# yl-jiang/YOLOSeries

Measured on AMD Instinct MI355X. Metric: images/sec (640x640) YOLOv5s train-step, higher is better.
Workload: dtype bf16; 1 GPU; YOLOv5s bf16 train step (fwd+loss+bwd+clip+SGD+EMA), batch 64/GPU x 640x640 synthetic COCO-80, random-init (BASELINE.json configs[1]); global_batch=64, parallelism=dp1

## Files before the change

yoloseries_amd/csrc/conv_dg2.hip:

```cpp
#include "common.h"
#include <stdlib.h>

namespace {

typedef __attribute__((ext_vector_type(4))) unsigned int u32x4_t;
typedef unsigned int u32x4_nt __attribute__((ext_vector_type(4)));

__device__ __forceinline__ uint4 dg_ld_nt16(const uint16_t* p) {
    u32x4_nt v = __builtin_nontemporal_load(reinterpret_cast<const u32x4_nt*>(p));
    return make_uint4(v.x, v.y, v.z, v.w);
}
__device__ __forceinline__ void dg_st_nt16(uint16_t* p, uint4 v) {
    u32x4_nt w = {v.x, v.y, v.z, v.w};
    __builtin_nontemporal_store(w, reinterpret_cast<u32x4_nt*>(p));
}

constexpr int DG_RPX1 = 128;
constexpr int dg_pmax(int pt) { return pt == 1 ? 168 : 304; }

struct Dg2K {
    const uint16_t* gz; int ldg, Nk;
    const uint16_t* w; int Ktot;
    uint16_t* out; int ld0, C;
    int B, Hg, Wg, Ho, Wo;
    int TH, TW, tx, ty, ntiles, nchunk, npatch;
    int accumulate;
    const uint16_t* z; int ldz; const float* ws; int wsC; float* part;
    unsigned gzbytes, wbytes;
};

template <int CT, int KC, int PT>
constexpr int dg_smem_bytes() {
    const int main_b = (dg_pmax(PT) + 9 * 32 * CT) * (KC + 8) * 2;
    const int stg_b = 2 * DG_RPX1 * PT * (32 * CT + 8) * 2;
    return (main_b > stg_b ? main_b : stg_b) + 2 * 32 * CT * 4;
}

template <int CT, int KC, int EPI, int PT>
__global__ __launch_bounds__(256 * CT, 1) void conv_dg2_kernel(const Dg2K p)
{
    constexpr int NT = 256 * CT;
    constexpr int DG_RPX = DG_RPX1 * PT;
    constexpr int DG_PMAX = dg_pmax(PT);
    constexpr int PITCH = KC + 8;
    constexpr int CHR = KC / 8;
    constexpr int CB = 32 * CT;
    constexpr int PPP = NT / CHR;
    constexpr int NPI = (DG_PMAX + PPP - 1) / PPP;
    constexpr int NWI = (9 * CB + PPP - 1) / PPP;
    constexpr int SP = CB + 8;
    constexpr int CPR = CB / 8;
    constexpr int NOI = 2 * DG_RPX * CPR / NT;
    constexpr unsigned OOB = 0x80000000u;
    constexpr int PATCH_BYTES = DG_PMAX * PITCH * 2;
    constexpr int STG_BYTES = 2 * DG_RPX * SP * 2;
    constexpr bool STG_IN_PATCH = STG_BYTES <= PATCH_BYTES;
    static_assert(NT % CPR == 0 && NOI == 4 * PT, "read-out mapping");

    extern __shared__ __attribute__((aligned(16))) unsigned char smem[];
    uint16_t* sP = reinterpret_cast<uint16_t*>(smem);
    uint16_t* sW = sP + DG_PMAX * PITCH;
    float* sStat = reinterpret_cast<float*>(smem + dg_smem_bytes<CT, KC, PT>() - 2 * CB * 4);
    uint16_t* sStg = reinterpret_cast<uint16_t*>(smem);

    const int t = threadIdx.x;
    const int lane = t & 63;
    const int wave = t >> 6;
    const int wq = wave & 3, wct = wave >> 2;
    const int c0 = blockIdx.y * CB;
    const int TWp = p.TW + 1;

    const __amdgpu_buffer_rsrc_t rsg = __builtin_amdgcn_make_buffer_rsrc((void*)p.gz, 0, p.gzbytes, 0x00020000);
    const __amdgpu_buffer_rsrc_t rsw = __builtin_amdgcn_make_buffer_rsrc((void*)p.w, 0, p.wbytes, 0x00020000);

    const int ch = t % CHR, row0 = t / CHR;
    unsigned woff[NWI];
#pragma unroll
    for (int j = 0; j < NWI; ++j) {
        const int row = row0 + j * PPP;
        const int tap = row / CB, c = row - tap * CB;
        woff[j] = row < 9 * CB ? (unsigned)((((size_t)(c0 + c) * p.Ktot) + tap * p.Nk + ch * 8) * 2) : OOB;
    }
    int ppij[NPI];
#pragma unroll
    for (int j = 0; j < NPI; ++j) {
        const int pp = row0 + j * PPP;
        const int pi = pp / TWp;
        ppij[j] = pp < p.npatch ? (pi << 8) | (pp - pi * TWp) : -1;
    }
    const int koff = (lane >> 5) * 8;
    int rpx[PT];
    const uint16_t* xbase[PT];
#pragma unroll
    for (int pt = 0; pt < PT; ++pt) {
        rpx[pt] = (wq * PT + pt) * 32 + (lane & 31);
        const bool rvalid = rpx[pt] < p.TH * p.TW;
        const int ri = rvalid ? rpx[pt] / p.TW : 0;
        const int rj = rvalid ? rpx[pt] - ri * p.TW : 0;
        xbase[pt] = sP + (ri * TWp + rj) * PITCH + koff;
    }
    const uint16_t* const wbase = sW + (wct * 32 + (lane & 31)) * PITCH + koff;

    if (EPI == 3) {
        for (int i = t; i < 2 * CB; i += NT) {
            const int which = i / CB, c = i - which * CB;
            sStat[i] = (c0 + c < p.C) ? p.ws[(size_t)which * p.wsC + c0 + c] : 0.f;
        }
    }
    float bs_[8], bq_[8];
#pragma unroll
    for (int e = 0; e < 8; ++e) { bs_[e] = 0.f; bq_[e] = 0.f; }

    u32x4_t rp[NPI], rw[NWI];
    const bool w_resident = STG_IN_PATCH && p.nchunk == 1;

    auto tile_origin = [&](int tile, int& b, int& i0, int& j0) {
        const int per = p.tx * p.ty;
        b = tile / per;
        const int r = tile - b * per;
        const int tyi = r / p.tx;
        i0 = tyi * p.TH; j0 = (r - tyi * p.tx) * p.TW;
    };
    auto load_regs = [&](int tile, int kc, bool with_w) {
        int b, i0, j0;
        tile_origin(tile, b, i0, j0);
        const int so = kc * KC * 2;
#pragma unroll
        for (int j = 0; j < NPI; ++j) {
            const int gi = i0 + (ppij[j] >> 8), gj = j0 + (ppij[j] & 0xff);
            const bool ok = ppij[j] >= 0 && gi < p.Hg && gj < p.Wg;
            const unsigned off = ok ? (unsigned)(((b * p.Hg + gi) * p.Wg + gj) * (p.ldg * 2) + ch * 16) : OOB;
            rp[j] = __builtin_amdgcn_raw_buffer_load_b128(rsg, off, so, 0);
        }
        if (with_w) {
#pragma unroll
            for (int j = 0; j < NWI; ++j) rw[j] = __builtin_amdgcn_raw_buffer_load_b128(rsw, woff[j], so, 0);
        }
    };
    auto store_regs = [&](bool with_w) {
        uint16_t* dp = sP + row0 * PITCH + ch * 8;
#pragma unroll
        for (int j = 0; j < NPI; ++j)
            if (row0 + j * PPP < DG_PMAX) *reinterpret_cast<u32x4_t*>(dp + j * PPP * PITCH) = rp[j];
        if (with_w) {
            uint16_t* dw = sW + row0 * PITCH + ch * 8;
#pragma unroll
            for (int j = 0; j < NWI; ++j)
                if (row0 + j * PPP < 9 * CB) *reinterpret_cast<u32x4_t*>(dw + j * PPP * PITCH) = rw[j];
        }
    };

    f32x16_t acc[4][PT];
    int tile = blockIdx.x;
    if (tile >= p.ntiles) return;
    load_regs(tile, 0, true);
    bool first = true;
    for (; tile < p.ntiles; tile += gridDim.x) {
#pragma unroll
        for (int q = 0; q < 4; ++q)
#pragma unroll
            for (int pt = 0; pt < PT; ++pt)
#pragma unroll
                for (int r = 0; r < 16; ++r) acc[q][pt][r] = 0.f;
        for (int kc = 0; kc < p.nchunk; ++kc) {
            const bool with_w = !w_resident || first;
            __syncthreads();
            store_regs(with_w);
            __syncthreads();
            first = false;
            {
                int nt = tile, nk = kc + 1;
                if (nk == p.nchunk) { nk = 0; nt = tile + gridDim.x; }
                if (nt < p.ntiles) load_regs(nt, nk, !w_resident);
            }
#pragma unroll
            for (int sh = 0; sh < 4; ++sh) {
                const int dy = sh >> 1, dx = sh & 1;
                bf16x8_t xf[PT][KC / 16];
#pragma unroll
                for (int pt = 0; pt < PT; ++pt)
#pragma unroll
                    for (int ks = 0; ks < KC / 16; ++ks)
                        xf[pt][ks] = __builtin_bit_cast(bf16x8_t, *reinterpret_cast<const uint4*>(xbase[pt] + (dy * TWp + dx) * PITCH + ks * 16));
#pragma unroll
                for (int a = 0; a < (dy ? 1 : 2); ++a) {
                    const int kh = dy ? 0 : 1 + a;
#pragma unroll
                    for (int b2 = 0; b2 < (dx ? 1 : 2); ++b2) {
                        const int kw = dx ? 0 : 1 + b2;
                        const int tap = kh * 3 + kw;
                        const int cls = (kh != 1 ? 2 : 0) + (kw != 1 ? 1 : 0);
#pragma unroll
                        for (int ks = 0; ks < KC / 16; ++ks) {
                            const bf16x8_t wf = __builtin_bit_cast(bf16x8_t, *reinterpret_cast<const uint4*>(wbase + tap * CB * PITCH + ks * 16));
#pragma unroll
                            for (int pt = 0; pt < PT; ++pt)
                                acc[cls][pt] = __builtin_amdgcn_mfma_f32_32x32x16_bf16(wf, xf[pt][ks], acc[cls][pt], 0, 0, 0);
                        }
                    }
                }
            }
        }

        int b, i0, j0;
        tile_origin(tile, b, i0, j0);
        const int cch = t % CPR;
        const int n = c0 + cch * 8;
#pragma unroll
        for (int ph = 0; ph < 2; ++ph) {
            int oidx[NOI];
            constexpr bool ZPRE = EPI == 3 && PT == 1;
            uint4 zpre[ZPRE ? NOI : 1];
#pragma unroll
            for (int it = 0; it < NOI; ++it) {
                const int row = t / CPR + it * (NT / CPR);
                const int r = row >> 1, pw = row & 1;
                const int i = r / p.TW, j = r - i * p.TW;
                const int gi = i0 + i, gj = j0 + j;
                const bool ok = r < p.TH * p.TW && gi < p.Hg && gj < p.Wg && n < p.C;
                oidx[it] = ok ? (b * p.Ho + 2 * gi + ph) * p.Wo + 2 * gj + pw : -1;
                if (ZPRE) {
                    zpre[it] = make_uint4(0, 0, 0, 0);
                    if (ok) zpre[it] = dg_ld_nt16(p.z + (size_t)oidx[it] * p.ldz + n);
                }
            }
            __syncthreads();
#pragma unroll
            for (int pw = 0; pw < 2; ++pw)
#pragma unroll
                for (int pt = 0; pt < PT; ++pt) {
                    uint16_t* dst = sStg + (rpx[pt] * 2 + pw) * SP + wct * 32 + 4 * (lane >> 5);
                    const f32x16_t& a = acc[ph * 2 + pw][pt];
#pragma unroll
                    for (int q = 0; q < 4; ++q) {
                        uint2 v;
                        v.x = pack2(a[4 * q + 0], a[4 * q + 1]);
                        v.y = pack2(a[4 * q + 2], a[4 * q + 3]);
                        *reinterpret_cast<uint2*>(dst + 8 * q) = v;
                    }
                }
            __syncthreads();
#pragma unroll
            for (int it = 0; it < NOI; ++it) {
                if (oidx[it] < 0) continue;
                const int row = t / CPR + it * (NT / CPR);
                uint4 v = *reinterpret_cast<const uint4*>(sStg + row * SP + cch * 8);
                uint16_t* dst = p.out + (size_t)oidx[it] * p.ld0 + n;
                if (p.accumulate) {
                    const uint4 ov = *reinterpret_cast<const uint4*>(dst);
                    float f[8], g0[8];
                    unpack8(v, f);
                    unpack8(ov, g0);
#pragma unroll
                    for (int e = 0; e < 8; ++e) f[e] += g0[e];
                    v = pack8(f);
                }
                if (EPI == 3) dg_st_nt16(dst, v);
                else *reinterpret_cast<uint4*>(dst) = v;
                if (EPI == 3) {
                    float g[8], z[8];
                    unpack8(v, g);
                    const uint4 zv = ZPRE ? zpre[it] : dg_ld_nt16(p.z + (size_t)oidx[it] * p.ldz + n);
                    unpack8(zv, z);
                    const float4 s0 = *reinterpret_cast<const float4*>(sStat + cch * 8);
                    const float4 s1 = *reinterpret_cast<const float4*>(sStat + cch * 8 + 4);
                    const float4 h0 = *reinterpret_cast<const float4*>(sStat + CB + cch * 8);
                    const float4 h1 = *reinterpret_cast<const float4*>(sStat + CB + cch * 8 + 4);
                    const float sc[8] = {s0.x, s0.y, s0.z, s0.w, s1.x, s1.y, s1.z, s1.w};
                    const float sh[8] = {h0.x, h0.y, h0.z, h0.w, h1.x, h1.y, h1.z, h1.w};
#pragma unroll
                    for (int e = 0; e < 8; ++e) {
                        const float a = z[e] * sc[e] + sh[e];
                        const float sg = sigmoid_fast(a);
                        const float dz = g[e] * (sg * (1.f + a * (1.f - sg)));
                        bs_[e] += dz; bq_[e] += dz * z[e];
                    }
                }
            }
        }
    }

    if (EPI == 3) {
        float* sRed = reinterpret_cast<float*>(smem);
        __syncthreads();
#pragma unroll
        for (int e = 0; e < 8; ++e) { sRed[t * 16 + e] = bs_[e]; sRed[t * 16 + 8 + e] = bq_[e]; }
        __syncthreads();
        for (int i = t; i < 2 * CB; i += NT) {
            const int which = i / CB, c = i - which * CB;
            float v = 0.f;
            for (int j = c / 8; j < NT; j += CPR) v += sRed[j * 16 + which * 8 + (c & 7)];
            if (c0 + c < p.C) p.part[((size_t)blockIdx.x * 2 + which) * p.C + c0 + c] = v;
        }
    }
}

bool dg2_geom(int Hg, int Wg, int pt, int* TH, int* TW, int* tx, int* ty)
{
    double best = -1.0;
    const int rpx = DG_RPX1 * pt;
    for (int tw = 4; tw <= 64; ++tw)
        for (int th = 1; th * tw <= rpx; ++th) {
            if ((th + 1) * (tw + 1) > dg_pmax(pt)) continue;
            const int nx = (Wg + tw - 1) / tw, ny = (Hg + th - 1) / th;
            double eff = (double)Hg * Wg / ((double)nx * ny * rpx);
            eff += 1e-4 * tw;
            if (eff > best) { best = eff; *TH = th; *TW = tw; *tx = nx; *ty = ny; }
        }
    return best > 0.0;
}

struct Dg2Plan { int ct, kc, pt, gx, gy; Dg2K k; };

bool dg2_plan(const yh_conv_desc* d, Dg2Plan* pl)
{
    if (d->mode != YH_CONV_DGRAD || d->nseg != 1 || d->seg[0].ups) return false;
    if (d->KH != 3 || d->KW != 3 || d->stride != 2 || d->pad != 1) return false;
    if (d->Ho != 2 * d->Hi || d->Wo != 2 * d->Wi) return false;
    if (d->bias || d->scale || d->shift || d->act != YH_ACT_NONE || d->res || d->nsplit < d->N || d->stats) return false;
    const int Nk = d->seg[0].C;
    if (Nk % 32 || d->N % 8) return false;
    const unsigned long gzb = ((unsigned long)d->B * d->Hi * d->Wi - 1) * d->seg[0].ld * 2 + (unsigned long)Nk * 2;
    const unsigned long wb = (unsigned long)d->Npad * 9 * Nk * 2;
    if (gzb >= (1ul << 31) || wb >= (1ul << 31)) return false;
    if ((unsigned long)d->B * d->Ho * d->Wo >= (1ul << 31)) return false;
    Dg2K& k = pl->k;
    pl->ct = d->N <= 32 ? 1 : 2;
    pl->kc = (Nk % 64 == 0 && d->tile_k != 32) ? 64 : 32;
    pl->pt = 1;
    if (!dg2_geom(d->Hi, d->Wi, pl->pt, &k.TH, &k.TW, &k.tx, &k.ty)) return false;
    const int cb = 32 * pl->ct;
    pl->gy = (d->N + cb - 1) / cb;
    if (pl->gy * cb > d->Npad) return false;
    k.gz = d->seg[0].ptr; k.ldg = d->seg[0].ld; k.Nk = Nk;
    k.w = d->w; k.Ktot = 9 * Nk;
    k.out = d->out0; k.ld0 = d->ld0; k.C = d->N;
    k.B = d->B; k.Hg = d->Hi; k.Wg = d->Wi; k.Ho = d->Ho; k.Wo = d->Wo;
    k.ntiles = d->B * k.tx * k.ty;
    k.nchunk = Nk / pl->kc;
    k.npatch = (k.TH + 1) * (k.TW + 1);
    k.accumulate = d->accumulate;
    k.z = d->bnr_z; k.ldz = d->bnr_ldz; k.ws = d->bnr_ws; k.wsC = d->bnr_C; k.part = d->bnr_part;
    k.gzbytes = (unsigned)gzb; k.wbytes = (unsigned)wb;
    int cap = (256 * (pl->ct == 1 ? 2 : 1)) / pl->gy;
    if (cap < 1) cap = 1;
    if (d->grid_cap > 0) cap = d->grid_cap;
    pl->gx = k.ntiles < cap ? k.ntiles : cap;
    return true;
}

}

int yh_dg2_rows(const yh_conv_desc* d)
{
    Dg2Plan pl;
    return dg2_plan(d, &pl) ? pl.gx : 0;
}

int yh_dg2_run(const yh_conv_desc* d, yh_stream stream, char* name_out, int name_len)
{
    Dg2Plan pl;
    YH_CHECK_ARG(dg2_plan(d, &pl), "yh_conv_igemm: algo 7 (stride-2 data-gradient kernel) is not eligible for this descriptor");
    const int epi = d->bnr_part ? 3 : 0;
    if (d->bnr_part)
        YH_CHECK_ARG(d->bnr_z && yh_aligned16(d->bnr_z) && d->bnr_ldz % 8 == 0 && d->bnr_ws && d->bnr_C >= d->N, "yh_conv_igemm: bad fused-reduction operands");
    if (name_out) { snprintf(name_out, name_len, "conv_dg2_kernel<%d, %d, %d, %d>", pl.ct, pl.kc, epi, pl.pt); return YH_OK; }
    hipStream_t st = (hipStream_t)stream;
    const dim3 grid(pl.gx, pl.gy), blk(256 * pl.ct);
#define YH_LAUNCH_DG2(CT_, KC_, PT_)                                                                                   \
    do {                                                                                                               \
        const int sm = dg_smem_bytes<CT_, KC_, PT_>();                                                                 \
        static YhDevOnce attr_set;                                                                                        \
        yh_lds_limit(attr_set, {{(const void*)conv_dg2_kernel<CT_, KC_, 0, PT_>, sm}, {(const void*)conv_dg2_kernel<CT_, KC_, 3, PT_>, sm}}); \
        if (epi == 3) conv_dg2_kernel<CT_, KC_, 3, PT_><<<grid, blk, sm, st>>>(pl.k);                                  \
        else          conv_dg2_kernel<CT_, KC_, 0, PT_><<<grid, blk, sm, st>>>(pl.k);                                  \
    } while (0)
    if (pl.ct == 1)      { if (pl.kc == 64) YH_LAUNCH_DG2(1, 64, 1); else YH_LAUNCH_DG2(1, 32, 1); }
    else                 { if (pl.kc == 64) YH_LAUNCH_DG2(2, 64, 1); else YH_LAUNCH_DG2(2, 32, 1); }
#undef YH_LAUNCH_DG2
    YH_CHECK_LAUNCH("yh_conv_igemm(dg2)");
    return YH_OK;
}
```

Measured before the change: 5485 images/sec.

## Add double-buffered direct-to-LDS DMA ring pipeline to stride-2 data-gradient conv

Adds a ring path to the stride-2 data-gradient kernel. It loads gradient patches and weights straight into LDS with buffer_load...lds in 32-channel sub-chunks, double-buffered and interleaved with the MFMA loop, using XOR-swizzled LDS addresses. The path is chosen at compile time when the output staging would not fit inside the patch buffer, and it uses separate LDS regions for staging. The aim is to overlap global loads with compute and remove register round-trips. The cost is larger LDS use, inline asm with m0 handling, and added probe and ablation hooks.

```diff
diff --git a/yoloseries_amd/csrc/conv_dg2.hip b/yoloseries_amd/csrc/conv_dg2.hip
--- a/yoloseries_amd/csrc/conv_dg2.hip
+++ b/yoloseries_amd/csrc/conv_dg2.hip
@@ -17,6 +17,20 @@
 
 constexpr int DG_RPX1 = 128;
 constexpr int dg_pmax(int pt) { return pt == 1 ? 168 : 304; }
+
+constexpr int DG_KS = 32;
+constexpr int DG_ROWB = DG_KS * 2;
+constexpr int DG_PPIECE = (dg_pmax(1) + 15) / 16;
+constexpr int dg_ring_buf(int ct) { return (DG_PPIECE + 18 * ct) * 1024; }
+constexpr int dg_ring_smem(int ct) { return 2 * dg_ring_buf(ct) + 2 * DG_RPX1 * (32 * ct + 8) * 2 + 2 * 32 * ct * 4; }
+
+__device__ __forceinline__ void dg_dma(unsigned lds, unsigned voff, const __amdgpu_buffer_rsrc_t rs, int soff) {
+    asm volatile("s_mov_b32 m0, %0\n\ts_nop 4\n\tbuffer_load_dwordx4 %1, %2, %3 offen lds" :: "s"(lds), "v"(voff), "s"(rs), "s"(soff) : "memory");
+}
+
+#ifdef YH_CONV_STAMPS
+__device__ long long g_dg2_stamps[64];
+#endif
 
 struct Dg2K {
     const uint16_t* gz; int ldg, Nk;
@@ -24,6 +38,7 @@
     uint16_t* out; int ld0, C;
     int B, Hg, Wg, Ho, Wo;
     int TH, TW, tx, ty, ntiles, nchunk, npatch;
+    int nsub;
     int accumulate;
     const uint16_t* z; int ldz; const float* ws; int wsC; float* part;
     unsigned gzbytes, wbytes;
@@ -36,8 +51,8 @@
     return (main_b > stg_b ? main_b : stg_b) + 2 * 32 * CT * 4;
 }
 
-template <int CT, int KC, int EPI, int PT>
-__global__ __launch_bounds__(256 * CT, 1) void conv_dg2_kernel(const Dg2K p)
+template <int CT, int KC, int EPI, int PT, bool RING>
+__device__ __forceinline__ void dg2_body(const Dg2K& p, unsigned char* const smem)
 {
     constexpr int NT = 256 * CT;
     constexpr int DG_RPX = DG_RPX1 * PT;
@@ -56,12 +71,21 @@
     constexpr int STG_BYTES = 2 * DG_RPX * SP * 2;
     constexpr bool STG_IN_PATCH = STG_BYTES <= PATCH_BYTES;
     static_assert(NT % CPR == 0 && NOI == 4 * PT, "read-out mapping");
-
-    extern __shared__ __attribute__((aligned(16))) unsigned char smem[];
+    static_assert(NT * 16 * 4 <= STG_BYTES || PT != 1, "the reduction scratch fits the output staging");
+    static_assert(!RING || PT == 1, "the ring deals one pixel tile per wave");
+    constexpr bool HAS_RING = RING, HAS_REG = !RING;
+    constexpr int NW = 4 * CT;
+    constexpr int RBUF = dg_ring_buf(CT);
+    constexpr int RW0 = DG_PPIECE * 1024;
+    constexpr int NWPIECE = 18 * CT;
+    constexpr int NPP = (DG_PPIECE + NW - 1) / NW, NWP = (NWPIECE + NW - 1) / NW;
+    constexpr bool ring = RING;
+
     uint16_t* sP = reinterpret_cast<uint16_t*>(smem);
     uint16_t* sW = sP + DG_PMAX * PITCH;
-    float* sStat = reinterpret_cast<float*>(smem + dg_smem_bytes<CT, KC, PT>() - 2 * CB * 4);
-    uint16_t* sStg = reinterpret_cast<uint16_t*>(smem);
+    unsigned char* const stg0 = smem + (ring ? 2 * RBUF : 0);
+    float* sStat = reinterpret_cast<float*>(ring ? stg0 + STG_BYTES : smem + dg_smem_bytes<CT, KC, PT>() - 2 * CB * 4);
+    uint16_t* sStg = reinterpret_cast<uint16_t*>(stg0);
 
     const int t = threadIdx.x;
     const int lane = t & 63;
@@ -100,6 +124,36 @@
         xbase[pt] = sP + (ri * TWp + rj) * PITCH + koff;
     }
     const uint16_t* const wbase = sW + (wct * 32 + (lane & 31)) * PITCH + koff;
+
+    const int wv = __builtin_amdgcn_readfirstlane(wave);
+    const int wfirst = (wv + NW - DG_PPIECE % NW) % NW;
+    const int lrow = lane >> 2, srcch = (lane & 3) ^ ((lane >> 4) & 3);
+    unsigned rwoff[NWP], rpoff[NPP];
+    int rppij[NPP];
+    unsigned xa[4], wa = 0;
+    if (HAS_RING) {
+#pragma unroll
+        for (int j = 0; j < NWP; ++j) {
+            const int i = wfirst + j * NW, row = i * 16 + lrow;
+            const int tap = row / CB, c = row - tap * CB;
+            rwoff[j] = (i < NWPIECE && c0 + c < p.C) ? (unsigned)((((size_t)(c0 + c) * p.Ktot) + tap * p.Nk + srcch * 8) * 2) : OOB;
+        }
+#pragma unroll
+        for (int j = 0; j < NPP; ++j) {
+            const int pp = (wv + j * NW) * 16 + lrow;
+            const int pi = pp / TWp;
+            rppij[j] = pp < p.npatch ? (pi << 8) | (pp - pi * TWp) : -1;
+            rpoff[j] = OOB;
+        }
+        const int rvalid = rpx[0] < p.TH * p.TW;
+        const int ri = rvalid ? rpx[0] / p.TW : 0, rj = rvalid ? rpx[0] - ri * p.TW : 0;
+#pragma unroll
+        for (int sh = 0; sh < 4; ++sh) {
+            const int xrow = (ri + (sh >> 1)) * TWp + rj + (sh & 1);
+            xa[sh] = (unsigned)(xrow * DG_ROWB + (((lane >> 5) ^ ((xrow >> 2) & 3)) << 4));
+        }
+        wa = (unsigned)(RW0 + (wct * 32 + (lane & 31)) * DG_ROWB + (((lane >> 5) ^ ((lane >> 2) & 3)) << 4));
+    }
 
     if (EPI == 3) {
         for (int i = t; i < 2 * CB; i += NT) {
@@ -150,10 +204,55 @@
         }
     };
 
+    const unsigned lds0 = (unsigned)(size_t)((__attribute__((address_space(3))) unsigned char*)smem);
+    int it_tile = blockIdx.x, it_s = 0;
+    auto ring_begin = [&]() -> bool {
+        if (it_tile >= p.ntiles) return false;
+        if (it_s == 0) {
+            int b, i0, j0;
+            tile_origin(it_tile, b, i0, j0);
+#pragma unroll
+            for (int j = 0; j < NPP; ++j) {
+                const int gi = i0 + (rppij[j] >> 8), gj = j0 + (rppij[j] & 0xff);
+                const bool ok = rppij[j] >= 0 && gi < p.Hg && gj < p.Wg;
+                rpoff[j] = ok ? (unsigned)(((b * p.Hg + gi) * p.Wg + gj) * (p.ldg * 2) + srcch * 16) : OOB;
+            }
+        }
+        return true;
+    };
+    auto ring_piece = [&](int j, unsigned la, int so) {
+        if (j < NPP) {
+            const int i = wv + j * NW;
+            if (i < DG_PPIECE) dg_dma(la + i * 1024, rpoff[j < NPP ? j : 0], rsg, so);
+        } else if (j < NPP + NWP) {
+            const int i = wfirst + (j - NPP) * NW;
+            if (i < NWPIECE) dg_dma(la + RW0 + i * 1024, rwoff[j < NPP ? 0 : j - NPP], rsw, so);
+        }
+    };
+    auto ring_end = [&]() { if (++it_s == p.nsub) { it_s = 0; it_tile += gridDim.x; } };
+#ifdef YH_CONV_STAMPS
+    long long st_mma = 0, st_wait = 0, st_bar = 0, st_epi = 0, st_n = 0;
+    const long long st_begin = __builtin_amdgcn_s_memtime();
+    long long st_t = st_begin;
+#define DG_STAMP(var) do { const long long now_ = __builtin_amdgcn_s_memtime(); var += now_ - st_t; st_t = now_; } while (0)
+#else
+#define DG_STAMP(var) do { } while (0)
+#endif
+
     f32x16_t acc[4][PT];
     int tile = blockIdx.x;
     if (tile >= p.ntiles) return;
-    load_regs(tile, 0, true);
+    int cur = 0;
+    if (ring) {
+        ring_begin();
+#pragma unroll
+        for (int j = 0; j < NPP + NWP; ++j) ring_piece(j, lds0, 0);
+        ring_end();
+        YH_VMCNT(0);
+        __syncthreads();
+    } else if (HAS_REG) {
+        load_regs(tile, 0, true);
+    }
     bool first = true;
     for (; tile < p.ntiles; tile += gridDim.x) {
 #pragma unroll
@@ -162,7 +261,49 @@
             for (int pt = 0; pt < PT; ++pt)
 #pragma unroll
                 for (int r = 0; r < 16; ++r) acc[q][pt][r] = 0.f;
-        for (int kc = 0; kc < p.nchunk; ++kc) {
+        DG_STAMP(st_epi);
+        if (HAS_RING && ring) for (int s = 0; s < p.nsub; ++s) {
+            const unsigned char* const bb = smem + cur * RBUF;
+            const bool more = ring_begin();
+            const unsigned la = lds0 + (unsigned)((cur ^ 1) * RBUF);
+            const int so = it_s * DG_ROWB;
+#pragma unroll
+            for (int sh = 0; sh < 4; ++sh) {
+                const int dy = sh >> 1, dx = sh & 1;
+                bf16x8_t xf[DG_KS / 16];
+#pragma unroll
+                for (int ks = 0; ks < DG_KS / 16; ++ks)
+                    xf[ks] = __builtin_bit_cast(bf16x8_t, *reinterpret_cast<const uint4*>(bb + (xa[sh] ^ (ks << 5))));
+#pragma unroll
+                for (int a = 0; a < (dy ? 1 : 2); ++a) {
+                    const int kh = dy ? 0 : 1 + a;
+#pragma unroll
+                    for (int b2 = 0; b2 < (dx ? 1 : 2); ++b2) {
+                        const int kw = dx ? 0 : 1 + b2;
+                        const int tap = kh * 3 + kw;
+                        const int cls = (kh != 1 ? 2 : 0) + (kw != 1 ? 1 : 0);
+#pragma unroll
+                        for (int ks = 0; ks < DG_KS / 16; ++ks) {
+                            const bf16x8_t wf = __builtin_bit_cast(bf16x8_t, *reinterpret_cast<const uint4*>(bb + (wa ^ (ks << 5)) + tap * CB * DG_ROWB));
+                            acc[cls][0] = __builtin_amdgcn_mfma_f32_32x32x16_bf16(wf, xf[ks], acc[cls][0], 0, 0, 0);
+                            const int m = ((sh == 0 ? 0 : sh == 1 ? 4 : sh == 2 ? 6 : 8) + a * (dx ? 1 : 2) + b2) * (DG_KS / 16) + ks;
+                            if (more) ring_piece(m, la, so);
+                        }
+                    }
+                }
+            }
+            if (more) ring_end();
+            DG_STAMP(st_mma);
+            YH_VMCNT(0);
+            DG_STAMP(st_wait);
+            __syncthreads();
+            DG_STAMP(st_bar);
+            cur ^= 1;
+#ifdef YH_CONV_STAMPS
+            ++st_n;
+#endif
+        }
+        if (HAS_REG && !ring) for (int kc = 0; kc < p.nchunk; ++kc) {
             const bool with_w = !w_resident || first;
             __syncthreads();
             store_regs(with_w);
@@ -280,8 +421,18 @@
         }
     }
 
+#ifdef YH_CONV_STAMPS
+    DG_STAMP(st_epi);
+    if (blockIdx.x == 0 && blockIdx.y == 0 && lane == 0) {
+        long long* o = g_dg2_stamps + wave * 8;
+        o[0] = st_mma; o[1] = st_wait; o[2] = st_bar; o[3] = 0; o[4] = st_epi; o[5] = st_n; o[6] = p.nsub;
+        o[7] = __builtin_amdgcn_s_memtime() - st_begin;
+    }
+#endif
+#undef DG_STAMP
+
     if (EPI == 3) {
-        float* sRed = reinterpret_cast<float*>(smem);
+        float* sRed = reinterpret_cast<float*>(sStg);
         __syncthreads();
 #pragma unroll
         for (int e = 0; e < 8; ++e) { sRed[t * 16 + e] = bs_[e]; sRed[t * 16 + 8 + e] = bq_[e]; }
@@ -293,6 +444,16 @@
             if (c0 + c < p.C) p.part[((size_t)blockIdx.x * 2 + which) * p.C + c0 + c] = v;
         }
     }
+}
+
+template <int CT, int KC, int PT>
+constexpr bool dg_has_reg() { return PT != 1 || 2 * DG_RPX1 * PT * (32 * CT + 8) <= dg_pmax(PT) * (KC + 8); }
+
+template <int CT, int KC, int EPI, int PT>
+__global__ __launch_bounds__(256 * CT, 1) void conv_dg2_kernel(const Dg2K p)
+{
+    extern __shared__ __attribute__((aligned(16))) unsigned char smem[];
+    dg2_body<CT, KC, EPI, PT, !dg_has_reg<CT, KC, PT>()>(p, smem);
 }
 
 bool dg2_geom(int Hg, int Wg, int pt, int* TH, int* TW, int* tx, int* ty)
@@ -338,6 +499,7 @@
     k.B = d->B; k.Hg = d->Hi; k.Wg = d->Wi; k.Ho = d->Ho; k.Wo = d->Wo;
     k.ntiles = d->B * k.tx * k.ty;
     k.nchunk = Nk / pl->kc;
+    k.nsub = Nk / DG_KS;
     k.npatch = (k.TH + 1) * (k.TW + 1);
     k.accumulate = d->accumulate;
     k.z = d->bnr_z; k.ldz = d->bnr_ldz; k.ws = d->bnr_ws; k.wsC = d->bnr_C; k.part = d->bnr_part;
@@ -367,9 +529,13 @@
     if (name_out) { snprintf(name_out, name_len, "conv_dg2_kernel<%d, %d, %d, %d>", pl.ct, pl.kc, epi, pl.pt); return YH_OK; }
     hipStream_t st = (hipStream_t)stream;
     const dim3 grid(pl.gx, pl.gy), blk(256 * pl.ct);
+    static const int abl = [] { const char* e = getenv("YH_DG2_ABL"); return e ? atoi(e) : 0; }();
+    if (abl & 1) pl.k.gzbytes = pl.k.wbytes = 0;
 #define YH_LAUNCH_DG2(CT_, KC_, PT_)                                                                                   \
     do {                                                                                                               \
-        const int sm = dg_smem_bytes<CT_, KC_, PT_>();                                                                 \
+        constexpr int sm_reg = dg_smem_bytes<CT_, KC_, PT_>(), sm_ring = dg_ring_smem(CT_);                            \
+        constexpr bool has_reg = dg_has_reg<CT_, KC_, PT_>();                                                          \
+        constexpr int sm = has_reg ? sm_reg : sm_ring;                                                                 \
         static YhDevOnce attr_set;                                                                                        \
         yh_lds_limit(attr_set, {{(const void*)conv_dg2_kernel<CT_, KC_, 0, PT_>, sm}, {(const void*)conv_dg2_kernel<CT_, KC_, 3, PT_>, sm}}); \
         if (epi == 3) conv_dg2_kernel<CT_, KC_, 3, PT_><<<grid, blk, sm, st>>>(pl.k);                                  \
@@ -381,3 +547,10 @@
     YH_CHECK_LAUNCH("yh_conv_igemm(dg2)");
     return YH_OK;
 }
+
+#ifdef YH_CONV_STAMPS
+extern "C" int yh_debug_read_dg2_stamps(long long* host_out64)
+{
+    return hipMemcpyFromSymbol(host_out64, HIP_SYMBOL(g_dg2_stamps), sizeof(long long) * 64) == hipSuccess ? 0 : -1;
+}
+#endif
```

Result: no change. 5483 images/sec (-0.0%).
